# KinWaiCheuk/ReconVAT

Hardware: AMD Instinct MI355X
Metric: training audio-sec/sec (node) (higher is better)
Workload: dtype f32; 1 GPU; ReconVAT UNet_Onset VAT=True reconstruction=True, per-GPU B_l=8 + B_ul=8 segments of 327680 samples (640 frames x 229 mel), Adam+StepLR, fp32; parallelism=dp1, hipgraph=True, two_stream_schedule=True, kernel_plan_table=644fe159bb9eb70e, kernel_plan_mode=table, vat_nan_flag=0

## Files before the change

reconvat_amd/csrc/conv.hip:

```cpp
#include "conv_band.h"
#include <mutex>

struct PackArgs {
    const float* w;
    float* out;
    int taps, kdim, ndim;
    int R, ntile_n, nchunk;
    long s_k, s_n;
    int flip;
    int scatter_cmid;
    long total;
    long wino0;
};

__device__ __forceinline__ void pack_wino_elem(const PackArgs& a, long idx) {
    const int R = a.R;
    int r = (int)(idx % R);
    long t = idx / R;
    int lane = (int)(t % 64); t /= 64;
    int nt = (int)(t % a.ntile_n); t /= a.ntile_n;
    int c = (int)(t % a.nchunk);
    int xi = (int)(t / a.nchunk);
    int k = c * 4 * R + (lane >> 4) * R + r;
    int n = nt * 16 + (lane & 15);
// ... 1411 lines not shown
        asm volatile("s_waitcnt vmcnt(0)" ::: "memory");
        if (!(ABL(a) & 8)) __syncthreads();
        prefetched = (row + 1 < row1) && (y + 1 < a.Hv);
#ifdef RV_ABLATION
        if (stamp) { const unsigned long long t = __builtin_amdgcn_s_memtime(); t_wait += t - t_mark; t_mark = t; if (row == row0) a.dbg[2] = t; }
#endif
        if (prefetched && !(ABL(a) & 4)) stage_next(b, y + 1, vb ^ 1);
#ifdef RV_ABLATION
        if (stamp) { const unsigned long long t = __builtin_amdgcn_s_memtime(); a.dbg[8] += t - t_mark; t_mark = t; }
#endif
        int slot_of[KH];
#pragma unroll
        for (int ky = 0; ky < KH; ++ky) slot_of[ky] = slot_of_row(y, ky);
        const float* vrow = vbuf + vb * Wv4 * CB;
        float vfA[TB], ufA[TAPS][TAW], vfB[TB], ufB[TAPS][TAW];
        auto ld = [&](float (&vf)[TB], float (&uf)[TAPS][TAW], const int x0) {
            const int x = x0 + g;
            if (ABL(a) & 2) {
#pragma unroll
                for (int tb = 0; tb < TB; ++tb) vf[tb] = (float)x0;
#pragma unroll
                for (int t = 0; t < TAPS; ++t)
#pragma unroll
                    for (int ta = 0; ta < TAW; ++ta) uf[t][ta] = (float)(x0 + t);
                return;
            }
#pragma unroll
            for (int tb = 0; tb < TB; ++tb) vf[tb] = vrow[x * CB + tb * 16 + i];
#pragma unroll
            for (int ky = 0; ky < KH; ++ky) {
                const float* ur = ubuf + slot_of[ky] * UP * CA + (S * x) * CA + i;
#pragma unroll
                for (int kx = 0; kx < KW; ++kx)
#pragma unroll
                    for (int ta = 0; ta < TAW; ++ta) {
#ifdef RV_ABLATION
                        if ((ABL(a) & 256) && ky * KW + kx >= 4) { uf[ky * KW + kx][ta] = 0.f; continue; }
#endif
                        uf[ky * KW + kx][ta] = ur[kx * CA + (hp * TAW + ta) * 16];
                    }
            }
        };
        auto mm = [&](const float (&vf)[TB], const float (&uf)[TAPS][TAW]) {
            if (ABL(a) & 1) {
#pragma unroll
                for (int t = 0; t < TAPS; ++t)
#pragma unroll
                    for (int ta = 0; ta < TAW; ++ta) acc[t][ta][0][0] += uf[t][ta] * vf[0] + vf[TB - 1];
                return;
            }
#ifdef RV_ABLATION
            if (ABL(a) & 256) {
                float vv[TB];
#pragma unroll
                for (int tb = 0; tb < TB; ++tb) vv[tb] = vf[tb];
                if (ABL(a) & 512) {
#pragma unroll
                    for (int q = 0; q < 14; ++q) asm volatile("v_add_f32 %0, %0, %1" : "+v"(vv[q % TB]) : "v"(uf[q % TAPS][0]));
                }
#pragma unroll
                for (int t = 0; t < 4; ++t)
#pragma unroll
                    for (int ta = 0; ta < TAW; ++ta)
#pragma unroll
                        for (int tb = 0; tb < TB; ++tb)
                            acc[t][ta][tb] = __builtin_amdgcn_mfma_f32_16x16x4f32(uf[t][ta], vv[tb], acc[t][ta][tb], 0, 0, 0);
                return;
            }
#endif
#pragma unroll
            for (int t = 0; t < TAPS; ++t)
#pragma unroll
                for (int ta = 0; ta < TAW; ++ta)
#pragma unroll
                    for (int tb = 0; tb < TB; ++tb)
                        acc[t][ta][tb] = __builtin_amdgcn_mfma_f32_16x16x4f32(uf[t][ta], vf[tb], acc[t][ta][tb], 0, 0, 0);
            if (do_bias) {
#pragma unroll
                for (int tb = 0; tb < TB; ++tb) accbs[tb] += vf[tb];
            }
        };
        auto interleave = [&]() {
#pragma unroll
            for (int k = 0; k < TAPS * TAW * TB; ++k) {
                __builtin_amdgcn_sched_group_barrier(0x008, 1, 0);
                if (k < TB + TAPS * TAW) __builtin_amdgcn_sched_group_barrier(0x100, 1, 0);
            }
        };
        constexpr int DX = 4 * NXG;
        if constexpr (BF) {
            for (int xb0 = xg * 16; xb0 < Wv4; xb0 += 16 * NXG) {
                const int x = xb0 + g;
                float vraw[TB][4], uraw[TAPS][TAW][4];
#pragma unroll
                for (int tb = 0; tb < TB; ++tb)
#pragma unroll
                    for (int e = 0; e < 4; ++e) vraw[tb][e] = vrow[(x + 4 * e) * CB + tb * 16 + i];
#pragma unroll
                for (int ky = 0; ky < KH; ++ky) {
                    const float* ur = ubuf + slot_of[ky] * UP * CA + (S * x) * CA + i;
#pragma unroll
                    for (int kx = 0; kx < KW; ++kx)
#pragma unroll
                        for (int ta = 0; ta < TAW; ++ta)
#pragma unroll
                            for (int e = 0; e < 4; ++e) uraw[ky * KW + kx][ta][e] = ur[(S * 4 * e + kx) * CA + (hp * TAW + ta) * 16];
                }
                s16x4 vb16[TB], ub16[TAPS][TAW];
#pragma unroll
                for (int tb = 0; tb < TB; ++tb) vb16[tb] = to_bf16x4((f32x4){vraw[tb][0], vraw[tb][1], vraw[tb][2], vraw[tb][3]});
#pragma unroll
                for (int t = 0; t < TAPS; ++t)
#pragma unroll
                    for (int ta = 0; ta < TAW; ++ta)
                        ub16[t][ta] = to_bf16x4((f32x4){uraw[t][ta][0], uraw[t][ta][1], uraw[t][ta][2], uraw[t][ta][3]});
#pragma unroll
                for (int t = 0; t < TAPS; ++t)
#pragma unroll
                    for (int ta = 0; ta < TAW; ++ta)
#pragma unroll
                        for (int tb = 0; tb < TB; ++tb)
                            acc[t][ta][tb] = __builtin_amdgcn_mfma_f32_16x16x16bf16_1k(ub16[t][ta], vb16[tb], acc[t][ta][tb], 0, 0, 0);
                if (do_bias) {
#pragma unroll
                    for (int tb = 0; tb < TB; ++tb) accbs[tb] += (vraw[tb][0] + vraw[tb][1]) + (vraw[tb][2] + vraw[tb][3]);
                }
            }
            continue;
        }
        const int xlast = Wv4 - 4;
        int x0 = xg * 4;
        if (x0 < Wv4) {
            ld(vfA, ufA, x0);
            for (;;) {
                const int x1 = x0 + DX;
                ld(vfB, ufB, min(x1, xlast));
                mm(vfA, ufA);
                interleave();
                if (x1 >= Wv4) break;
                x0 = x1 + DX;
                ld(vfA, ufA, min(x0, xlast));
                mm(vfB, ufB);
                interleave();
                if (x0 >= Wv4) break;
            }
        }
#ifdef RV_ABLATION
        if (stamp) t_comp += __builtin_amdgcn_s_memtime() - t_mark;
#endif
    }
#ifdef RV_ABLATION
    if (stamp) { a.dbg[6] = t_wait; a.dbg[7] = t_comp; }
#endif
    TS(3);
    if (do_bias) {
#pragma unroll
        for (int tb = 0; tb < TB; ++tb) {
            float sb = accbs[tb];
            sb += __shfl_xor(sb, 16, 64);
            sb += __shfl_xor(sb, 32, 64);
            accb[tb] = (f32x4){sb, sb, sb, sb};
        }
    }
    if (ABL(a) & 32) { if (acc[0][0][0][0] == 123.456f) a.part[0] = accbs[0]; return; }
    constexpr int NVEC = TAPS * TAW * TB + TB;
    static_assert((NXG & (NXG - 1)) == 0, "x groups must be a power of two");
#pragma unroll
    for (int half = NXG / 2; half >= 1; half >>= 1) {
        f32x4* fold = reinterpret_cast<f32x4*>(smem) + (hp * (NXG / 2) + (xg & (half - 1))) * NVEC * 64 + lane;
        __syncthreads();
        if (xg >= half && xg < 2 * half) {
            int q = 0;
#pragma unroll
            for (int t = 0; t < TAPS; ++t)
#pragma unroll
                for (int ta = 0; ta < TAW; ++ta)
#pragma unroll
                    for (int tb = 0; tb < TB; ++tb) fold[(q++) * 64] = acc[t][ta][tb];
#pragma unroll
            for (int tb = 0; tb < TB; ++tb) fold[(q++) * 64] = accb[tb];
        }
        __syncthreads();
        if (xg < half) {
            int q = 0;
#pragma unroll
            for (int t = 0; t < TAPS; ++t)
#pragma unroll
                for (int ta = 0; ta < TAW; ++ta)
#pragma unroll
                    for (int tb = 0; tb < TB; ++tb) acc[t][ta][tb] += fold[(q++) * 64];
#pragma unroll
            for (int tb = 0; tb < TB; ++tb) accb[tb] += fold[(q++) * 64];
        }
    }
    TS(4);
    if (xg != 0) return;
    float* dst = a.part + (long)blockIdx.x * a.pstride;
#ifdef RV_ABLATION
    if (ABL(a) & 2048) {
        dst = a.part;
#pragma unroll
        for (int t = 0; t < TAPS; ++t)
#pragma unroll
            for (int ta = 0; ta < TAW; ++ta)
#pragma unroll
                for (int tb = 0; tb < TB; ++tb) {
                    const int bb = b0 + tb * 16 + i;
#pragma unroll
                    for (int r = 0; r < 4; ++r) {
                        const int aa = a0 + (hp * TAW + ta) * 16 + 4 * g + r;
                        if (aa < a.Ca && bb < a.Cb) atomicAdd(&dst[((long)t * a.Ca + aa) * a.Cb + bb], acc[t][ta][tb][r]);
                    }
                }
        return;
    }
#endif
#pragma unroll
    for (int t = 0; t < TAPS; ++t)
#pragma unroll
        for (int ta = 0; ta < TAW; ++ta)
#pragma unroll
            for (int tb = 0; tb < TB; ++tb) {
                const int bb = b0 + tb * 16 + i;
#pragma unroll
                for (int r = 0; r < 4; ++r) {
                    const int aa = a0 + (hp * TAW + ta) * 16 + 4 * g + r;
                    if (aa < a.Ca && bb < a.Cb) dst[((long)t * a.Ca + aa) * a.Cb + bb] = acc[t][ta][tb][r];
                }
            }
    if (do_bias && g == 0) {
#pragma unroll
        for (int tb = 0; tb < TB; ++tb) {
            const int bb = b0 + tb * 16 + i;
            if (bb < a.Cb) dst[(long)TAPS * a.Ca * a.Cb + bb] = accb[tb][0];
        }
    }
    TS(5);
#undef TS
}

template <int C> __device__ __forceinline__ int wgw_pos(int X, int c) {
    return C == 32 ? X * 32 + ((((c >> 4) ^ ((X >> 1) & 1)) << 4) | (c & 15)) : (X ^ ((X >> 1) & 1)) * 16 + c;
}

template <int TA, int TB, int NW>
__global__ __launch_bounds__(NW * 64) void wgrad_wino_k(WgradArgs a) {
    constexpr int CA = TA * 16, CB = TB * 16;
    constexpr int NH = (NW == 8 && TA == 2 && TB == 2) ? 2 : 1;
    constexpr int TAW = TA / NH, NXG = NW / NH;
    constexpr int C4A = CA / 4, C4B = CB / 4;
    constexpr int PPA = 64 / C4A, PPB = 64 / C4B;
    constexpr int NSLOT = 6;
    extern __shared__ __attribute__((aligned(16))) float smem[];
    const int tid = threadIdx.x, lane = tid & 63;
    const int wave = __builtin_amdgcn_readfirstlane(tid >> 6);
    const int i = lane & 15, g = lane >> 4;
    const int ga = blockIdx.y / a.ngb, gb = blockIdx.y - ga * a.ngb;
    const int a0 = ga * CA, b0 = gb * CB;
    const int H2 = a.Hv >> 1;
    const int npairs = a.B * H2;
    const int pair0 = blockIdx.x * a.rows_per_wave;
    const int pair1 = min(pair0 + a.rows_per_wave, npairs);
    const int WT = (a.Wv + 1) >> 1, WT4 = (WT + 3) & ~3;
    const int UPp = ((2 * WT4 + 2 + PPA - 1) / PPA) * PPA;
    const int VPp = ((2 * WT4 + PPB - 1) / PPB) * PPB;
    float* ubuf = smem;
    float* vbuf = smem + NSLOT * UPp * CA;
    const int hp = wave / NXG, xg = (wave + (NH == 2 ? 2 * hp : 0)) % NXG;

    f32x4 acc[16][TAW][TB];
#pragma unroll
    for (int xi = 0; xi < 16; ++xi)
#pragma unroll
        for (int x = 0; x < TAW; ++x)
#pragma unroll
            for (int y = 0; y < TB; ++y) acc[xi][x][y] = (f32x4){0.f, 0.f, 0.f, 0.f};
    f32x4 accb[TB];
    float accbs[TB];
#pragma unroll
    for (int y = 0; y < TB; ++y) { accb[y] = (f32x4){0.f, 0.f, 0.f, 0.f}; accbs[y] = 0.f; }
    const bool do_bias = a.want_bias && ga == 0 && hp == 0;
    const int ca_valid = min(CA, a.Ca - a0), cb_valid = min(CB, a.Cb - b0);

    constexpr unsigned OOB = 0x40000000u;
    constexpr int MAXP = 4;
    const int upl = lane / C4A, uql = lane - upl * C4A;
    const int vpl = lane / C4B, vql = lane - vpl * C4B;
    auto u_off = [&](int k) -> unsigned {
        const int Xs = k * PPA + upl;
        const int X = CA == 32 ? Xs : (Xs ^ ((Xs >> 1) & 1));
        const int q = CA == 32 ? (uql ^ (4 * ((X >> 1) & 1))) : uql;
        const int x = X - 1;
        return ((unsigned)x < (unsigned)a.Wu && q * 4 < ca_valid) ? (unsigned)(x * a.u_ld + q * 4) * 4u : OOB;
    };
    auto v_off = [&](int k) -> unsigned {
        const int Xs = k * PPB + vpl;
        const int X = CB == 32 ? Xs : (Xs ^ ((Xs >> 1) & 1));
        const int q = CB == 32 ? (vql ^ (4 * ((X >> 1) & 1))) : vql;
        return (X < a.Wv && q * 4 < cb_valid) ? (unsigned)(X * a.v_ld + q * 4) * 4u : OOB;
    };
    unsigned u_goff[MAXP], v_goff[MAXP];
#pragma unroll
    for (int j = 0; j < MAXP; ++j) { u_goff[j] = u_off(wave + NW * j); v_goff[j] = v_off(wave + NW * j); }
    auto dma_urow = [&](int b, int r, int slot) {
        float* dst0 = ubuf + slot * UPp * CA;
        int bl;
        const int sg = wgrad_seg_of(a, b, bl);
        const rv_rsrc_t rs_u = rv_make_rsrc(a.Useg[sg], a.u_bytes);
        const unsigned base = (unsigned)r < (unsigned)a.Hu ? (unsigned)(((bl * a.Hu + r) * a.Wu) * a.u_ld + a0) * 4u : OOB;
#pragma unroll
        for (int j = 0; j < MAXP; ++j) {
            const int k = wave + NW * j;
            if (k * PPA >= UPp) break;
            rv_buf_lds16(rs_u, dst0 + k * PPA * CA, u_goff[j] + base);
        }
        for (int k = wave + NW * MAXP; k * PPA < UPp; k += NW) rv_buf_lds16(rs_u, dst0 + k * PPA * CA, u_off(k) + base);
    };
    auto dma_vrow = [&](int b, int y, int vslot) {
        float* dst0 = vbuf + vslot * VPp * CB;
        int bl;
        const int sg = wgrad_seg_of(a, b, bl);
        const rv_rsrc_t rs_v = rv_make_rsrc(a.Vseg[sg], a.v_bytes);
        const unsigned base = (unsigned)(((bl * a.Hv + y) * a.Wv) * a.v_ld + b0) * 4u;
#pragma unroll
        for (int j = 0; j < MAXP; ++j) {
            const int k = wave + NW * j;
            if (k * PPB >= VPp) break;
            rv_buf_lds16(rs_v, dst0 + k * PPB * CB, v_goff[j] + base);
        }
        for (int k = wave + NW * MAXP; k * PPB < VPp; k += NW) rv_buf_lds16(rs_v, dst0 + k * PPB * CB, v_off(k) + base);
    };
    auto uslot = [&](int r) -> int { return (r + 1 + NSLOT) % NSLOT; };
    auto stage_full = [&](int b, int yp, int vb) {
#pragma unroll
        for (int e = 0; e < 4; ++e) dma_urow(b, 2 * yp - 1 + e, uslot(2 * yp - 1 + e));
        dma_vrow(b, 2 * yp, vb * 2);
        dma_vrow(b, 2 * yp + 1, vb * 2 + 1);
    };
    auto stage_next = [&](int b, int yp, int vb) {
        dma_urow(b, 2 * yp + 1, uslot(2 * yp + 1));
        dma_urow(b, 2 * yp + 2, uslot(2 * yp + 2));
        dma_vrow(b, 2 * yp, vb * 2);
        dma_vrow(b, 2 * yp + 1, vb * 2 + 1);
    };

    int uoff[4][TAW], voff[2][TB];
#pragma unroll
    for (int ec = 0; ec < 4; ++ec)
#pragma unroll
        for (int ta = 0; ta < TAW; ++ta) uoff[ec][ta] = wgw_pos<CA>(2 * g + ec, (hp * TAW + ta) * 16 + i);
#pragma unroll
    for (int dx = 0; dx < 2; ++dx)
#pragma unroll
        for (int tb = 0; tb < TB; ++tb) voff[dx][tb] = wgw_pos<CB>(2 * g + dx, tb * 16 + i);

    bool prefetched = false;
    for (int pair = pair0; pair < pair1; ++pair) {
        const int b = pair / H2, yp = pair - b * H2;
        const int vb = pair & 1;
        if (!prefetched) {
            __syncthreads();
            stage_full(b, yp, vb);
        }
        asm volatile("s_waitcnt vmcnt(0)" ::: "memory");
        __syncthreads();
        prefetched = (pair + 1 < pair1) && (yp + 1 < H2);
        if (prefetched) stage_next(b, yp + 1, vb ^ 1);
        const float* urow[4];
#pragma unroll
        for (int e = 0; e < 4; ++e) urow[e] = ubuf + uslot(2 * yp - 1 + e) * UPp * CA;
        const float* vrow0 = vbuf + (vb * 2) * VPp * CB;
        const float* vrow1 = vrow0 + VPp * CB;
        constexpr int USTEP = 2 * 4 * NXG * CA, VSTEP = 2 * 4 * NXG * CB, KMAX = 8;
        const float* up[4][4][TAW];
        const float* vp[4][TB];
#pragma unroll
        for (int er = 0; er < 4; ++er)
#pragma unroll
            for (int ec = 0; ec < 4; ++ec)
#pragma unroll
                for (int ta = 0; ta < TAW; ++ta) up[er][ec][ta] = urow[er] + 2 * (xg * 4) * CA + uoff[ec][ta];
#pragma unroll
        for (int dx = 0; dx < 2; ++dx)
#pragma unroll
            for (int tb = 0; tb < TB; ++tb) {
                vp[dx][tb] = vrow0 + 2 * (xg * 4) * CB + voff[dx][tb];
                vp[2 + dx][tb] = vrow1 + 2 * (xg * 4) * CB + voff[dx][tb];
            }
        auto kstep = [&](const int uo, const int vo) __attribute__((always_inline)) {
            float d[16][TAW], y[4][TB];
#pragma unroll
            for (int er = 0; er < 4; ++er)
#pragma unroll
                for (int ec = 0; ec < 4; ++ec)
#pragma unroll
                    for (int ta = 0; ta < TAW; ++ta) d[er * 4 + ec][ta] = up[er][ec][ta][uo];
#pragma unroll
            for (int e = 0; e < 4; ++e)
#pragma unroll
                for (int tb = 0; tb < TB; ++tb) y[e][tb] = vp[e][tb][vo];
#pragma unroll
            for (int ta = 0; ta < TAW; ++ta) {
#pragma unroll
                for (int cc = 0; cc < 4; ++cc) {
                    const float e0 = d[cc][ta], e1 = d[4 + cc][ta], e2 = d[8 + cc][ta], e3 = d[12 + cc][ta];
                    d[cc][ta] = e0 - e2; d[4 + cc][ta] = e1 + e2; d[8 + cc][ta] = e2 - e1; d[12 + cc][ta] = e1 - e3;
                }
#pragma unroll
                for (int rr = 0; rr < 4; ++rr) {
                    const float e0 = d[4 * rr][ta], e1 = d[4 * rr + 1][ta], e2 = d[4 * rr + 2][ta], e3 = d[4 * rr + 3][ta];
                    d[4 * rr][ta] = e0 - e2; d[4 * rr + 1][ta] = e1 + e2; d[4 * rr + 2][ta] = e2 - e1; d[4 * rr + 3][ta] = e1 - e3;
                }
            }
            float q[16][TB];
#pragma unroll
            for (int tb = 0; tb < TB; ++tb) {
                const float y00 = y[0][tb], y01 = y[1][tb], y10 = y[2][tb], y11 = y[3][tb];
                const float t[4][2] = {{y00, y01}, {y00 + y10, y01 + y11}, {y00 - y10, y01 - y11}, {-y10, -y11}};
#pragma unroll
                for (int r = 0; r < 4; ++r) {
                    q[4 * r][tb] = t[r][0]; q[4 * r + 1][tb] = t[r][0] + t[r][1]; q[4 * r + 2][tb] = t[r][0] - t[r][1]; q[4 * r + 3][tb] = -t[r][1];
                }
                if (do_bias) accbs[tb] += q[5][tb];
            }
#pragma unroll
            for (int xi = 0; xi < 16; ++xi)
#pragma unroll
                for (int ta = 0; ta < TAW; ++ta)
#pragma unroll
                    for (int tb = 0; tb < TB; ++tb)
                        acc[xi][ta][tb] = __builtin_amdgcn_mfma_f32_16x16x4f32(d[xi][ta], q[xi][tb], acc[xi][ta][tb], 0, 0, 0);
        };
        const int nk = (WT4 - xg * 4 + 4 * NXG - 1) / (4 * NXG);
        sfor<0, KMAX>([&](auto sc) {
            constexpr int S = decltype(sc)::value;
            if (S < nk) kstep(S * USTEP, S * VSTEP);
        });
        for (int sk = KMAX; sk < nk; ++sk) kstep(sk * USTEP, sk * VSTEP);
    }
    if (do_bias) {
#pragma unroll
        for (int tb = 0; tb < TB; ++tb) {
            float sb = accbs[tb];
            sb += __shfl_xor(sb, 16, 64);
            sb += __shfl_xor(sb, 32, 64);
            accb[tb] = (f32x4){sb, sb, sb, sb};
        }
    }
    if (ABL(a) & 32) { if (acc[0][0][0][0] == 123.456f) a.part[0] = accbs[0]; return; }
    f32x4 tapv[9][TAW][TB];
#pragma unroll
    for (int ta = 0; ta < TAW; ++ta)
#pragma unroll
        for (int tb = 0; tb < TB; ++tb) {
            f32x4 t[3][4];
#pragma unroll
            for (int cc = 0; cc < 4; ++cc) {
                const f32x4 h = 0.5f * (acc[4 + cc][ta][tb] + acc[8 + cc][ta][tb]);
                t[0][cc] = acc[cc][ta][tb] + h;
                t[1][cc] = 0.5f * (acc[4 + cc][ta][tb] - acc[8 + cc][ta][tb]);
                t[2][cc] = h + acc[12 + cc][ta][tb];
            }
#pragma unroll
            for (int ky = 0; ky < 3; ++ky) {
                const f32x4 h = 0.5f * (t[ky][1] + t[ky][2]);
                tapv[ky * 3 + 0][ta][tb] = t[ky][0] + h;
                tapv[ky * 3 + 1][ta][tb] = 0.5f * (t[ky][1] - t[ky][2]);
                tapv[ky * 3 + 2][ta][tb] = h + t[ky][3];
            }
        }
    constexpr int NVEC = 9 * TAW * TB + TB;
    static_assert((NXG & (NXG - 1)) == 0, "x groups must be a power of two");
#pragma unroll
    for (int half = NXG / 2; half >= 1; half >>= 1) {
        f32x4* fold = reinterpret_cast<f32x4*>(smem) + (hp * (NXG / 2) + (xg & (half - 1))) * NVEC * 64 + lane;
        __syncthreads();
        if (xg >= half && xg < 2 * half) {
            int qn = 0;
#pragma unroll
            for (int t = 0; t < 9; ++t)
#pragma unroll
                for (int ta = 0; ta < TAW; ++ta)
#pragma unroll
                    for (int tb = 0; tb < TB; ++tb) fold[(qn++) * 64] = tapv[t][ta][tb];
#pragma unroll
            for (int tb = 0; tb < TB; ++tb) fold[(qn++) * 64] = accb[tb];
        }
        __syncthreads();
        if (xg < half) {
            int qn = 0;
#pragma unroll
            for (int t = 0; t < 9; ++t)
#pragma unroll
                for (int ta = 0; ta < TAW; ++ta)
#pragma unroll
                    for (int tb = 0; tb < TB; ++tb) tapv[t][ta][tb] += fold[(qn++) * 64];
#pragma unroll
            for (int tb = 0; tb < TB; ++tb) accb[tb] += fold[(qn++) * 64];
        }
    }
    if (xg != 0) return;
    float* dst = a.part + (long)blockIdx.x * a.pstride;
#pragma unroll
    for (int t = 0; t < 9; ++t)
#pragma unroll
        for (int ta = 0; ta < TAW; ++ta)
#pragma unroll
            for (int tb = 0; tb < TB; ++tb) {
                const int bb = b0 + tb * 16 + i;
#pragma unroll
                for (int r = 0; r < 4; ++r) {
                    const int aa = a0 + (hp * TAW + ta) * 16 + 4 * g + r;
                    if (aa < a.Ca && bb < a.Cb) dst[((long)t * a.Ca + aa) * a.Cb + bb] = tapv[t][ta][tb][r];
                }
            }
    if (do_bias && g == 0) {
#pragma unroll
        for (int tb = 0; tb < TB; ++tb) {
            const int bb = b0 + tb * 16 + i;
            if (bb < a.Cb) dst[(long)9 * a.Ca * a.Cb + bb] = accb[tb][0];
        }
    }
}

template <int CA, int CB, int KH, int KW, int S, int P>
__global__ __launch_bounds__(256) void wgrad_small_k(WgradArgs a) {
    constexpr int TAPS = KH * KW;
    constexpr bool SPLIT_B = CB >= CA;
    constexpr int CS = SPLIT_B ? CB : CA;
    constexpr int Q = CS >= 4 ? 4 : CS;
    constexpr int LPP = CS / Q;
    constexpr int PPW = 64 / LPP;
    constexpr int CAL = SPLIT_B ? CA : Q, CBL = SPLIT_B ? Q : CB;
    const int lane = threadIdx.x & 63, wave = threadIdx.x >> 6;
    const int ps = lane / LPP, cq = lane - ps * LPP;
    const int a_off = SPLIT_B ? 0 : cq * Q, b_off = SPLIT_B ? cq * Q : 0;
    const int pw = blockIdx.x * 4 + wave;
    if (pw >= a.nparts) return;
    float acc[TAPS][CAL][CBL];
    float accb[CBL];
#pragma unroll
    for (int t = 0; t < TAPS; ++t)
#pragma unroll
        for (int x = 0; x < CAL; ++x)
#pragma unroll
            for (int y = 0; y < CBL; ++y) acc[t][x][y] = 0.f;
#pragma unroll
    for (int y = 0; y < CBL; ++y) accb[y] = 0.f;
    const unsigned npix = (unsigned)(a.B * a.Hv * a.Wv);
    const unsigned per = (npix + a.nparts - 1) / a.nparts;
    const unsigned p0 = (unsigned)pw * per, p1 = min(p0 + per, npix);
    const bool vvec = (CBL % 4 == 0) && (a.v_ld % 4 == 0) && ((((uintptr_t)a.V) & 15) == 0);
    const bool uvec = (CAL % 4 == 0) && (a.u_ld % 4 == 0) && ((((uintptr_t)a.U) & 15) == 0);
    for (unsigned p = p0 + ps; p < p1; p += PPW) {
        const int b = (int)fastdiv(p, a.fd_vplane);
        const unsigned rem = p - (unsigned)b * (unsigned)(a.Hv * a.Wv);
        const int y = (int)fastdiv(rem, a.fd_wv), x = (int)rem - y * a.Wv;
        float v[CBL];
        const float* vp = a.V + (long)p * a.v_ld + b_off;
        if (CBL % 4 == 0 && vvec) {
#pragma unroll
            for (int c = 0; c < CBL; c += 4) {
                const f32x4 q = *reinterpret_cast<const f32x4*>(vp + c);
                v[c] = q[0]; v[c + 1] = q[1]; v[c + 2] = q[2]; v[c + 3] = q[3];
            }
        } else {
#pragma unroll
            for (int c = 0; c < CBL; ++c) v[c] = vp[c];
        }
#pragma unroll
        for (int c = 0; c < CBL; ++c) accb[c] += v[c];
#pragma unroll
        for (int ky = 0; ky < KH; ++ky)
#pragma unroll
            for (int kx = 0; kx < KW; ++kx) {
                int iy = y * S - P + ky, ix = x * S - P + kx;
                const bool inside = (unsigned)iy < (unsigned)a.Hu && (unsigned)ix < (unsigned)a.Wu;
                const float* up = a.U + (inside ? (((long)b * a.Hu + iy) * a.Wu + ix) * a.u_ld : 0L) + a_off;
                float u[CAL];
                if (CAL % 4 == 0 && uvec) {
#pragma unroll
                    for (int c = 0; c < CAL; c += 4) {
                        const f32x4 q = *reinterpret_cast<const f32x4*>(up + c);
                        u[c] = inside ? q[0] : 0.f; u[c + 1] = inside ? q[1] : 0.f; u[c + 2] = inside ? q[2] : 0.f; u[c + 3] = inside ? q[3] : 0.f;
                    }
                } else {
#pragma unroll
                    for (int ca = 0; ca < CAL; ++ca) u[ca] = inside ? up[ca] : 0.f;
                }
#pragma unroll
                for (int ca = 0; ca < CAL; ++ca)
#pragma unroll
                    for (int cb = 0; cb < CBL; ++cb)
                        acc[ky * KW + kx][ca][cb] = fmaf(u[ca], v[cb], acc[ky * KW + kx][ca][cb]);
            }
    }
    auto fold = [&](float s_) {
#pragma unroll
        for (int o = 32; o >= LPP; o >>= 1) s_ += __shfl_xor(s_, o, 64);
        return s_;
    };
    float* dst = a.part + (long)pw * a.pstride;
#pragma unroll
    for (int t = 0; t < TAPS; ++t)
#pragma unroll
        for (int ca = 0; ca < CAL; ++ca)
#pragma unroll
            for (int cb = 0; cb < CBL; ++cb) {
                const float s_ = fold(acc[t][ca][cb]);
                if (ps == 0) dst[((long)t * CA + a_off + ca) * CB + b_off + cb] = s_;
            }
#pragma unroll
    for (int cb = 0; cb < CBL; ++cb) {
        const float s_ = fold(accb[cb]);
        if (ps == 0 && a.want_bias && (SPLIT_B || cq == 0)) dst[(long)TAPS * CA * CB + b_off + cb] = s_;
    }
}

template <int CB>
__global__ __launch_bounds__(256) void wgrad_small_sw_k(WgradArgs a, int rows, int nstrip, int nband) {
    constexpr int CA = 8, LPP = 2, PXW = 32;
    const int lane = threadIdx.x & 63, wave = threadIdx.x >> 6;
    const int q = lane % LPP, col = lane / LPP;
    const int pw = blockIdx.x * 4 + wave;
    if (pw >= a.nparts) return;
    int id = pw;
    const int strip = id % nstrip; id /= nstrip;
    const int band = id % nband;
    const int b = id / nband;
    const int x = strip * PXW + col;
    const bool colok = x < a.Wv;
    const int y0 = band * rows, y1 = min(y0 + rows, a.Hv);
    const int cx[3] = {min(max(x - 1, 0), a.Wu - 1), min(x, a.Wu - 1), min(x + 1, a.Wu - 1)};
    const bool okx[3] = {colok && x - 1 >= 0, colok, colok && x + 1 < a.Wu};
    const float* img = a.U + (long)b * a.Hu * a.Wu * a.u_ld + 4 * q;
    const float* vimg = a.V + (long)b * a.Hv * a.Wv * a.v_ld;
    float acc[9][4][CB], accb[CB];
#pragma unroll
    for (int t = 0; t < 9; ++t)
#pragma unroll
        for (int c = 0; c < 4; ++c)
#pragma unroll
            for (int cb = 0; cb < CB; ++cb) acc[t][c][cb] = 0.f;
#pragma unroll
    for (int cb = 0; cb < CB; ++cb) accb[cb] = 0.f;
    auto load_raw = [&](f32x4 (&r)[3], int iy) {
        const float* rowp = img + (long)min(max(iy, 0), a.Hu - 1) * a.Wu * a.u_ld;
#pragma unroll
        for (int kx = 0; kx < 3; ++kx) r[kx] = *reinterpret_cast<const f32x4*>(rowp + (long)cx[kx] * a.u_ld);
    };
    auto mask_row = [&](f32x4 (&r)[3], int iy) {
        const bool oky = iy >= 0 && iy < a.Hu;
#pragma unroll
        for (int kx = 0; kx < 3; ++kx)
#pragma unroll
            for (int c = 0; c < 4; ++c) r[kx][c] = (oky && okx[kx]) ? r[kx][c] : 0.f;
    };
    auto load_v = [&](float (&v)[CB], int y) {
        const float* vp = vimg + ((long)min(y, a.Hv - 1) * a.Wv + min(x, a.Wv - 1)) * a.v_ld;
#pragma unroll
        for (int cb = 0; cb < CB; ++cb) v[cb] = vp[cb];
    };
    f32x4 win[3][3], nxt[3];
    float v[CB], vn[CB];
    load_raw(win[0], y0 - 1); load_raw(win[1], y0); load_raw(win[2], y0 + 1);
    load_v(v, y0);
    mask_row(win[0], y0 - 1); mask_row(win[1], y0); mask_row(win[2], y0 + 1);
    for (int y = y0; y < y1; ++y) {
        load_raw(nxt, y + 2);
        load_v(vn, y + 1);
#pragma unroll
        for (int cb = 0; cb < CB; ++cb) {
            const float vv = colok ? v[cb] : 0.f;
            if (q == 0) accb[cb] += vv;
#pragma unroll
            for (int ky = 0; ky < 3; ++ky)
#pragma unroll
                for (int kx = 0; kx < 3; ++kx)
#pragma unroll
                    for (int c = 0; c < 4; ++c) acc[ky * 3 + kx][c][cb] = fmaf(win[ky][kx][c], vv, acc[ky * 3 + kx][c][cb]);
        }
        mask_row(nxt, y + 2);
#pragma unroll
        for (int kx = 0; kx < 3; ++kx) { win[0][kx] = win[1][kx]; win[1][kx] = win[2][kx]; win[2][kx] = nxt[kx]; }
#pragma unroll
        for (int cb = 0; cb < CB; ++cb) v[cb] = vn[cb];
    }
    auto fold = [&](float s_) {
#pragma unroll
        for (int o = 32; o >= LPP; o >>= 1) s_ += __shfl_xor(s_, o, 64);
        return s_;
    };
    float* dst = a.part + (long)pw * a.pstride;
#pragma unroll
    for (int t = 0; t < 9; ++t)
#pragma unroll
        for (int c = 0; c < 4; ++c)
#pragma unroll
            for (int cb = 0; cb < CB; ++cb) {
                const float s_ = fold(acc[t][c][cb]);
                if (col == 0) dst[((long)t * CA + 4 * q + c) * CB + cb] = s_;
            }
#pragma unroll
    for (int cb = 0; cb < CB; ++cb) {
        float s_ = accb[cb];
#pragma unroll
        for (int o = 32; o >= 1; o >>= 1) s_ += __shfl_xor(s_, o, 64);
        if (lane == 0 && a.want_bias) dst[(long)9 * CA * CB + cb] = s_;
    }
}

__global__ __launch_bounds__(256) void wgrad_cin1_k(WgradArgs a, int rows, int nstrip, int nband) {
    constexpr int CB = 16, LPP = 4, PXW = 16;
    const int lane = threadIdx.x & 63, wave = threadIdx.x >> 6;
    const int q = lane % LPP, col = lane / LPP;
    const int pw = blockIdx.x * 4 + wave;
    if (pw >= a.nparts) return;
    int id = pw;
    const int strip = id % nstrip; id /= nstrip;
    const int band = id % nband;
    const int b = id / nband;
    const int x = strip * PXW + col;
    const bool colok = x < a.Wv;
    const int y0 = band * rows, y1 = min(y0 + rows, a.Hv);
    const int cx[3] = {min(max(x - 1, 0), a.Wu - 1), min(x, a.Wu - 1), min(x + 1, a.Wu - 1)};
    const bool okx[3] = {colok && x - 1 >= 0, colok, colok && x + 1 < a.Wu};
    const float* img = a.U + (long)b * a.Hu * a.Wu * a.u_ld;
    const float* vimg = a.V + (long)b * a.Hv * a.Wv * a.v_ld + 4 * q;
    f32x4 acc[9], accb = (f32x4){0.f, 0.f, 0.f, 0.f};
#pragma unroll
    for (int t = 0; t < 9; ++t) acc[t] = (f32x4){0.f, 0.f, 0.f, 0.f};
    auto load_raw = [&](float (&r)[3], int iy) {
        const float* rowp = img + (long)min(max(iy, 0), a.Hu - 1) * a.Wu * a.u_ld;
#pragma unroll
        for (int kx = 0; kx < 3; ++kx) r[kx] = rowp[(long)cx[kx] * a.u_ld];
    };
    auto mask_row = [&](float (&r)[3], int iy) {
        const bool oky = iy >= 0 && iy < a.Hu;
#pragma unroll
        for (int kx = 0; kx < 3; ++kx) r[kx] = (oky && okx[kx]) ? r[kx] : 0.f;
    };
    auto load_v = [&](int y) -> f32x4 {
        return *reinterpret_cast<const f32x4*>(vimg + ((long)min(y, a.Hv - 1) * a.Wv + min(x, a.Wv - 1)) * a.v_ld);
    };
    constexpr int PD = 3;
    float win[3][3], nxt[3], pre[PD][3];
    f32x4 vq[PD];
    load_raw(win[0], y0 - 1); load_raw(win[1], y0); load_raw(win[2], y0 + 1);
    f32x4 v = load_v(y0);
#pragma unroll
    for (int d = 0; d < PD; ++d) { load_raw(pre[d], y0 + 2 + d); vq[d] = load_v(y0 + 1 + d); }
    mask_row(win[0], y0 - 1); mask_row(win[1], y0); mask_row(win[2], y0 + 1);
    for (int y = y0; y < y1; ++y) {
#pragma unroll
        for (int kx = 0; kx < 3; ++kx) {
            nxt[kx] = pre[0][kx];
#pragma unroll
// ... 967 lines not shown
```

Baseline: 16610 audio-s/s.

## Strength-reduce wgrad Winograd row staging and fold sign flips into epilogue

```diff
diff --git a/reconvat_amd/csrc/conv.hip b/reconvat_amd/csrc/conv.hip
--- a/reconvat_amd/csrc/conv.hip
+++ b/reconvat_amd/csrc/conv.hip
@@ -1737,75 +1737,87 @@
     unsigned u_goff[MAXP], v_goff[MAXP];
 #pragma unroll
     for (int j = 0; j < MAXP; ++j) { u_goff[j] = u_off(wave + NW * j); v_goff[j] = v_off(wave + NW * j); }
-    auto dma_urow = [&](int b, int r, int slot) {
-        float* dst0 = ubuf + slot * UPp * CA;
-        int bl;
-        const int sg = wgrad_seg_of(a, b, bl);
-        const rv_rsrc_t rs_u = rv_make_rsrc(a.Useg[sg], a.u_bytes);
-        const unsigned base = (unsigned)r < (unsigned)a.Hu ? (unsigned)(((bl * a.Hu + r) * a.Wu) * a.u_ld + a0) * 4u : OOB;
+    const int nju = max(0, (UPp / PPA - wave + NW - 1) / NW), njv = max(0, (VPp / PPB - wave + NW - 1) / NW);
+    const int USLOT = UPp * CA, VSLOT = VPp * CB;
+    const unsigned urow_b = (unsigned)(a.Wu * a.u_ld) * 4u, vrow_b = (unsigned)(a.Wv * a.v_ld) * 4u;
+    auto dma_urow = [&](const rv_rsrc_t rs_u, const unsigned rowbase, const bool inside, const int slot_off) {
+        float* dst0 = ubuf + slot_off;
+        const unsigned base = inside ? rowbase : OOB;
 #pragma unroll
         for (int j = 0; j < MAXP; ++j) {
-            const int k = wave + NW * j;
-            if (k * PPA >= UPp) break;
-            rv_buf_lds16(rs_u, dst0 + k * PPA * CA, u_goff[j] + base);
+            if (j >= nju) break;
+            rv_buf_lds16(rs_u, dst0 + (wave + NW * j) * PPA * CA, u_goff[j] + base);
         }
         for (int k = wave + NW * MAXP; k * PPA < UPp; k += NW) rv_buf_lds16(rs_u, dst0 + k * PPA * CA, u_off(k) + base);
     };
-    auto dma_vrow = [&](int b, int y, int vslot) {
-        float* dst0 = vbuf + vslot * VPp * CB;
-        int bl;
-        const int sg = wgrad_seg_of(a, b, bl);
-        const rv_rsrc_t rs_v = rv_make_rsrc(a.Vseg[sg], a.v_bytes);
-        const unsigned base = (unsigned)(((bl * a.Hv + y) * a.Wv) * a.v_ld + b0) * 4u;
+    auto dma_vrow = [&](const rv_rsrc_t rs_v, const unsigned base, const int slot_off) {
+        float* dst0 = vbuf + slot_off;
 #pragma unroll
         for (int j = 0; j < MAXP; ++j) {
-            const int k = wave + NW * j;
-            if (k * PPB >= VPp) break;
-            rv_buf_lds16(rs_v, dst0 + k * PPB * CB, v_goff[j] + base);
+            if (j >= njv) break;
+            rv_buf_lds16(rs_v, dst0 + (wave + NW * j) * PPB * CB, v_goff[j] + base);
         }
         for (int k = wave + NW * MAXP; k * PPB < VPp; k += NW) rv_buf_lds16(rs_v, dst0 + k * PPB * CB, v_off(k) + base);
     };
-    auto uslot = [&](int r) -> int { return (r + 1 + NSLOT) % NSLOT; };
-    auto stage_full = [&](int b, int yp, int vb) {
-#pragma unroll
-        for (int e = 0; e < 4; ++e) dma_urow(b, 2 * yp - 1 + e, uslot(2 * yp - 1 + e));
-        dma_vrow(b, 2 * yp, vb * 2);
-        dma_vrow(b, 2 * yp + 1, vb * 2 + 1);
-    };
-    auto stage_next = [&](int b, int yp, int vb) {
-        dma_urow(b, 2 * yp + 1, uslot(2 * yp + 1));
-        dma_urow(b, 2 * yp + 2, uslot(2 * yp + 2));
-        dma_vrow(b, 2 * yp, vb * 2);
-        dma_vrow(b, 2 * yp + 1, vb * 2 + 1);
-    };
 
     int uoff[4][TAW], voff[2][TB];
 #pragma unroll
     for (int ec = 0; ec < 4; ++ec)
 #pragma unroll
-        for (int ta = 0; ta < TAW; ++ta) uoff[ec][ta] = wgw_pos<CA>(2 * g + ec, (hp * TAW + ta) * 16 + i);
+        for (int ta = 0; ta < TAW; ++ta) uoff[ec][ta] = 2 * (xg * 4) * CA + wgw_pos<CA>(2 * g + ec, (hp * TAW + ta) * 16 + i);
 #pragma unroll
     for (int dx = 0; dx < 2; ++dx)
 #pragma unroll
-        for (int tb = 0; tb < TB; ++tb) voff[dx][tb] = wgw_pos<CB>(2 * g + dx, tb * 16 + i);
+        for (int tb = 0; tb < TB; ++tb) voff[dx][tb] = 2 * (xg * 4) * CB + wgw_pos<CB>(2 * g + dx, tb * 16 + i);
+#pragma unroll
+    for (int ec = 0; ec < 4; ++ec)
+#pragma unroll
+        for (int ta = 0; ta < TAW; ++ta) asm volatile("" : "+v"(uoff[ec][ta]));
+#pragma unroll
+    for (int dx = 0; dx < 2; ++dx)
+#pragma unroll
+        for (int tb = 0; tb < TB; ++tb) asm volatile("" : "+v"(voff[dx][tb]));
+    const int nk = (WT4 - xg * 4 + 4 * NXG - 1) / (4 * NXG);
+
+    int bl = 0, yp = 0, sg = 0;
+    if (pair0 < pair1) {
+        const int b = pair0 / H2;
+        yp = pair0 - b * H2;
+        sg = wgrad_seg_of(a, b, bl);
+    }
+    rv_rsrc_t rs_u = rv_make_rsrc(a.Useg[sg], a.u_bytes), rs_v = rv_make_rsrc(a.Vseg[sg], a.v_bytes);
+    unsigned ubase = (unsigned)(((bl * a.Hu + 2 * yp - 1) * a.Wu) * a.u_ld + a0) * 4u;
+    unsigned vbase = (unsigned)(((bl * a.Hv + 2 * yp) * a.Wv) * a.v_ld + b0) * 4u;
+    int ringA = ((2 * yp) % NSLOT) * USLOT;
+    int ringB = ringA + 2 * USLOT >= NSLOT * USLOT ? ringA - 4 * USLOT : ringA + 2 * USLOT;
+    int ringC = ringB + 2 * USLOT >= NSLOT * USLOT ? ringB - 4 * USLOT : ringB + 2 * USLOT;
+    int vcur = (pair0 & 1) * 2 * VSLOT, vnxt = 2 * VSLOT - vcur;
+    const unsigned Hu_u = (unsigned)a.Hu;
 
     bool prefetched = false;
     for (int pair = pair0; pair < pair1; ++pair) {
-        const int b = pair / H2, yp = pair - b * H2;
-        const int vb = pair & 1;
+        const int r0 = 2 * yp - 1;
         if (!prefetched) {
             __syncthreads();
-            stage_full(b, yp, vb);
+            dma_urow(rs_u, ubase, (unsigned)r0 < Hu_u, ringA);
+            dma_urow(rs_u, ubase + urow_b, (unsigned)(r0 + 1) < Hu_u, ringA + USLOT);
+            dma_urow(rs_u, ubase + 2 * urow_b, (unsigned)(r0 + 2) < Hu_u, ringB);
+            dma_urow(rs_u, ubase + 3 * urow_b, (unsigned)(r0 + 3) < Hu_u, ringB + USLOT);
+            dma_vrow(rs_v, vbase, vcur);
+            dma_vrow(rs_v, vbase + vrow_b, vcur + VSLOT);
         }
         asm volatile("s_waitcnt vmcnt(0)" ::: "memory");
         __syncthreads();
         prefetched = (pair + 1 < pair1) && (yp + 1 < H2);
-        if (prefetched) stage_next(b, yp + 1, vb ^ 1);
-        const float* urow[4];
-#pragma unroll
-        for (int e = 0; e < 4; ++e) urow[e] = ubuf + uslot(2 * yp - 1 + e) * UPp * CA;
-        const float* vrow0 = vbuf + (vb * 2) * VPp * CB;
-        const float* vrow1 = vrow0 + VPp * CB;
+        if (prefetched) {
+            dma_urow(rs_u, ubase + 4 * urow_b, (unsigned)(r0 + 4) < Hu_u, ringC);
+            dma_urow(rs_u, ubase + 5 * urow_b, (unsigned)(r0 + 5) < Hu_u, ringC + USLOT);
+            dma_vrow(rs_v, vbase + 2 * vrow_b, vnxt);
+            dma_vrow(rs_v, vbase + 3 * vrow_b, vnxt + VSLOT);
+        }
+        const float* urow[4] = {ubuf + ringA, ubuf + ringA + USLOT, ubuf + ringB, ubuf + ringB + USLOT};
+        const float* vrow0 = vbuf + vcur;
+        const float* vrow1 = vrow0 + VSLOT;
         constexpr int USTEP = 2 * 4 * NXG * CA, VSTEP = 2 * 4 * NXG * CB, KMAX = 8;
         const float* up[4][4][TAW];
         const float* vp[4][TB];
@@ -1814,13 +1826,13 @@
 #pragma unroll
             for (int ec = 0; ec < 4; ++ec)
 #pragma unroll
-                for (int ta = 0; ta < TAW; ++ta) up[er][ec][ta] = urow[er] + 2 * (xg * 4) * CA + uoff[ec][ta];
+                for (int ta = 0; ta < TAW; ++ta) up[er][ec][ta] = urow[er] + uoff[ec][ta];
 #pragma unroll
         for (int dx = 0; dx < 2; ++dx)
 #pragma unroll
             for (int tb = 0; tb < TB; ++tb) {
-                vp[dx][tb] = vrow0 + 2 * (xg * 4) * CB + voff[dx][tb];
-                vp[2 + dx][tb] = vrow1 + 2 * (xg * 4) * CB + voff[dx][tb];
+                vp[dx][tb] = vrow0 + voff[dx][tb];
+                vp[2 + dx][tb] = vrow1 + voff[dx][tb];
             }
         auto kstep = [&](const int uo, const int vo) __attribute__((always_inline)) {
             float d[16][TAW], y[4][TB];
@@ -1851,11 +1863,12 @@
 #pragma unroll
             for (int tb = 0; tb < TB; ++tb) {
                 const float y00 = y[0][tb], y01 = y[1][tb], y10 = y[2][tb], y11 = y[3][tb];
-                const float t[4][2] = {{y00, y01}, {y00 + y10, y01 + y11}, {y00 - y10, y01 - y11}, {-y10, -y11}};
-#pragma unroll
-                for (int r = 0; r < 4; ++r) {
-                    q[4 * r][tb] = t[r][0]; q[4 * r + 1][tb] = t[r][0] + t[r][1]; q[4 * r + 2][tb] = t[r][0] - t[r][1]; q[4 * r + 3][tb] = -t[r][1];
+                const float t[3][2] = {{y00, y01}, {y00 + y10, y01 + y11}, {y00 - y10, y01 - y11}};
+#pragma unroll
+                for (int r = 0; r < 3; ++r) {
+                    q[4 * r][tb] = t[r][0]; q[4 * r + 1][tb] = t[r][0] + t[r][1]; q[4 * r + 2][tb] = t[r][0] - t[r][1]; q[4 * r + 3][tb] = t[r][1];
                 }
+                q[12][tb] = y10; q[13][tb] = y10 + y11; q[14][tb] = y11 - y10; q[15][tb] = y11;
                 if (do_bias) accbs[tb] += q[5][tb];
             }
 #pragma unroll
@@ -1866,12 +1879,26 @@
                     for (int tb = 0; tb < TB; ++tb)
                         acc[xi][ta][tb] = __builtin_amdgcn_mfma_f32_16x16x4f32(d[xi][ta], q[xi][tb], acc[xi][ta][tb], 0, 0, 0);
         };
-        const int nk = (WT4 - xg * 4 + 4 * NXG - 1) / (4 * NXG);
+        int nkp = nk;
+        asm volatile("" : "+s"(nkp));
         sfor<0, KMAX>([&](auto sc) {
             constexpr int S = decltype(sc)::value;
-            if (S < nk) kstep(S * USTEP, S * VSTEP);
+            if (S < nkp) kstep(S * USTEP, S * VSTEP);
         });
-        for (int sk = KMAX; sk < nk; ++sk) kstep(sk * USTEP, sk * VSTEP);
+        for (int sk = KMAX; sk < nkp; ++sk) kstep(sk * USTEP, sk * VSTEP);
+        { const int t = ringA; ringA = ringB; ringB = ringC; ringC = t; }
+        { const int t = vcur; vcur = vnxt; vnxt = t; }
+        ubase += 2 * urow_b; vbase += 2 * vrow_b;
+        if (++yp == H2) {
+            yp = 0;
+            if (++bl == a.Bseg && sg + 1 < a.nseg) {
+                bl = 0; ++sg;
+                rs_u = rv_make_rsrc(a.Useg[sg], a.u_bytes); rs_v = rv_make_rsrc(a.Vseg[sg], a.v_bytes);
+            }
+            ubase = (unsigned)(((bl * a.Hu - 1) * a.Wu) * a.u_ld + a0) * 4u;
+            vbase = (unsigned)(((bl * a.Hv) * a.Wv) * a.v_ld + b0) * 4u;
+            ringA = 0; ringB = 2 * USLOT; ringC = 4 * USLOT;
+        }
     }
     if (do_bias) {
 #pragma unroll
@@ -1888,6 +1915,8 @@
     for (int ta = 0; ta < TAW; ++ta)
 #pragma unroll
         for (int tb = 0; tb < TB; ++tb) {
+            acc[3][ta][tb] = -acc[3][ta][tb]; acc[7][ta][tb] = -acc[7][ta][tb]; acc[11][ta][tb] = -acc[11][ta][tb];
+            acc[12][ta][tb] = -acc[12][ta][tb]; acc[13][ta][tb] = -acc[13][ta][tb];
             f32x4 t[3][4];
 #pragma unroll
             for (int cc = 0; cc < 4; ++cc) {
```

New measurement: 16690 audio-s/s, median of 6. No clear change (+0.5%).
